# oxylusengine/Oxylus

Measured on NVIDIA H100. Metric: meshlet_instances_culled_per_s, higher is better.
Workload: dtype f32

## Files before the change

### oxylus_b200/csrc/kernels_cull.cuh

```cuda
#pragma once
#include "oxc_filtered.cuh"
#include "oxc_tma.cuh"

namespace oxc {

#ifndef OXC_CULL_MESHES_THREADS
#define OXC_CULL_MESHES_THREADS 64
#endif
constexpr int CULL_MESHES_THREADS = OXC_CULL_MESHES_THREADS;
constexpr int CULL_THREADS = 256;
#ifndef OXC_CULL_ITEMS
#define OXC_CULL_ITEMS 2
#endif
#ifndef OXC_CULL_MIN_BLOCKS
#define OXC_CULL_MIN_BLOCKS 3
#endif
constexpr int CULL_ITEMS = OXC_CULL_ITEMS;
constexpr int CULL_TILE = CULL_THREADS * CULL_ITEMS;

struct MeshesParams {
  const OxcMesh* meshes;
  OxcMeshInstance* mesh_instances;
  const OxcTransformWorld* transforms;
  InstCull* inst;
  InstGeom* geom;
  const float* lod_aabb;
  uint32_t* counts;
  uint32_t* block_sums;
  uint32_t first, count;
  uint32_t flags;
  int select;
  OxcCullCamera cam;
  const OxcCullCamera* cam_dev;
};

__global__ void __launch_bounds__(CULL_MESHES_THREADS) k_cull_meshes(const __grid_constant__ MeshesParams pp) {
  const MeshesParams& p = pp;
  const OxcCullCamera& cam = pp.cam_dev ? *pp.cam_dev : pp.cam;
  const uint32_t local = blockIdx.x * CULL_MESHES_THREADS + threadIdx.x;
  uint32_t meshlet_count = 0;
  if (local < p.count) {
    const uint32_t mi = p.first + local;
    OxcMeshInstance inst = p.mesh_instances[mi];
    const OxcMesh* mesh = &p.meshes[inst.mesh_index];
    const float* world = p.transforms[inst.transform_index].world;
    float w[16];
#pragma unroll
    for (int k = 0; k < 4; k++) {
      const float4 c = __ldg(reinterpret_cast<const float4*>(world) + k);
      w[k * 4 + 0] = c.x; w[k * 4 + 1] = c.y; w[k * 4 + 2] = c.z; w[k * 4 + 3] = c.w;
    }
    float4 rows[4], planes[6];
    mul_mm_rows(cam.projection_view, w, rows);
    frustum_planes(rows, planes);
// ... 68 lines not shown
    if (p.select) {
      InstGeom g;
      g.meshlets = reinterpret_cast<const OxcMeshlet*>(lod->meshlets);
      g.local_triangle_indices = reinterpret_cast<const uint32_t*>(lod->local_triangle_indices);
      g.indirect_vertex_indices = reinterpret_cast<const uint32_t*>(lod->indirect_vertex_indices);
      g.vertex_positions = reinterpret_cast<const uint2*>(mesh->vertex_positions);
      g.vertex_normals = reinterpret_cast<const uint32_t*>(mesh->vertex_normals);
      g.texture_coords = reinterpret_cast<const uint32_t*>(mesh->texture_coords);
      g.transform_index = inst.transform_index;
      g.vertex_count = mesh->vertex_count;
      g.pad[0] = g.pad[1] = 0;
      p.geom[mi] = g;
      p.counts[local] = meshlet_count;
    }
  }
  if (!p.select) return;
  __shared__ uint32_t warp_sums[CULL_MESHES_THREADS / 32];
  uint32_t v = meshlet_count;
#pragma unroll
  for (int o = 16; o > 0; o >>= 1) v += __shfl_xor_sync(0xffffffffu, v, o);
  if ((threadIdx.x & 31) == 0) warp_sums[threadIdx.x >> 5] = v;
  __syncthreads();
  if (threadIdx.x == 0) {
    uint32_t s = 0;
#pragma unroll
    for (int k = 0; k < CULL_MESHES_THREADS / 32; k++) s += warp_sums[k];
    p.block_sums[blockIdx.x] = s;
  }
}

__global__ void __launch_bounds__(CULL_MESHES_THREADS) k_count_prefix_meshlets(const __grid_constant__ MeshesParams p, uint32_t* id_base) {
  const OxcCullCamera& cam = p.cam_dev ? *p.cam_dev : p.cam;
  const uint32_t mi = blockIdx.x * CULL_MESHES_THREADS + threadIdx.x;
  uint32_t meshlet_count = 0;
  if (mi < p.first) {
    const OxcMeshInstance inst = p.mesh_instances[mi];
    const OxcMesh* mesh = &p.meshes[inst.mesh_index];
    const float* world = p.transforms[inst.transform_index].world;
    float w[16];
#pragma unroll
    for (int k = 0; k < 16; k++) w[k] = world[k];
    float4 rows[4], planes[6];
    mul_mm_rows(cam.projection_view, w, rows);
// ... 50 lines not shown
      }
    }
  } else bad = true;
#pragma unroll
  for (int a = 0; a < 3; a++)
#pragma unroll
    for (int o = 16; o > 0; o >>= 1) {
      mn[a] = fminf(mn[a], __shfl_xor_sync(0xffffffffu, mn[a], o));
      mx[a] = fmaxf(mx[a], __shfl_xor_sync(0xffffffffu, mx[a], o));
    }
  bad = __any_sync(0xffffffffu, bad);
  if (lane == 0) {
    float* o = out + (size_t)w * 6;
    if (bad) { o[0] = o[1] = o[2] = 1.0f; o[3] = o[4] = o[5] = -1.0f; }
    else { o[0] = mn[0]; o[1] = mn[1]; o[2] = mn[2]; o[3] = mx[0]; o[4] = mx[1]; o[5] = mx[2]; }
  }
}

__global__ void __launch_bounds__(1024) k_scan_block_sums(uint32_t* block_sums, uint32_t n_blocks,
                                                          OxcMeshletInstanceVisibility* vis,
                                                          OxcDispatchIndirectCommand* cmd, uint32_t capacity, uint32_t* status) {
  __shared__ uint32_t warp_tot[32];
  __shared__ uint32_t carry_s;
  if (threadIdx.x == 0) carry_s = 0;
  __syncthreads();
  for (uint32_t base = 0; base < n_blocks; base += 1024) {
    const uint32_t i = base + threadIdx.x;
    const uint32_t v = i < n_blocks ? block_sums[i] : 0u;
    uint32_t inc = v;
#pragma unroll
    for (int o = 1; o < 32; o <<= 1) {
      const uint32_t t = __shfl_up_sync(0xffffffffu, inc, o);
      if ((threadIdx.x & 31) >= o) inc += t;
    }
    if ((threadIdx.x & 31) == 31) warp_tot[threadIdx.x >> 5] = inc;
    __syncthreads();
    if (threadIdx.x < 32) {
      uint32_t w = warp_tot[threadIdx.x], winc = w;
#pragma unroll
      for (int o = 1; o < 32; o <<= 1) {
        const uint32_t t = __shfl_up_sync(0xffffffffu, winc, o);
        if (threadIdx.x >= o) winc += t;
      }
      warp_tot[threadIdx.x] = winc - w;
    }
    __syncthreads();
    const uint32_t carry = carry_s;
    const uint32_t excl = carry + warp_tot[threadIdx.x >> 5] + inc - v;
    if (i < n_blocks) block_sums[i] = excl;
    __syncthreads();
    if (threadIdx.x == 1023) carry_s = excl + v;
    __syncthreads();
  }
  if (threadIdx.x == 0) {
    uint32_t total = carry_s;
    if (total > capacity) {
      total = capacity;
      atomicOr(status, (uint32_t)OXC_STATUS_MESHLET_OVERFLOW);
    }
    vis->total_visible_meshlet_instances = total;
    vis->early_visible_meshlet_instances = 0;
    vis->late_visible_meshlet_instances = 0;
    cmd->x = (total + 63u) / 64u;
    cmd->y = 1;
    cmd->z = 1;
  }
}

constexpr int EXPAND_SPLIT = 8;
__global__ void __launch_bounds__(CULL_MESHES_THREADS) k_expand_meshlet_instances(const uint32_t* __restrict__ counts,
                                                                                 const uint32_t* __restrict__ block_offsets,
                                                                                 uint32_t first, uint32_t count,
                                                                                 OxcMeshletInstance* out, uint32_t capacity, uint2* slabs) {
  __shared__ uint32_t offs[CULL_MESHES_THREADS];
  __shared__ uint32_t cnts[CULL_MESHES_THREADS];
  __shared__ uint32_t warp_tot[CULL_MESHES_THREADS / 32];
  const uint32_t block = blockIdx.x / EXPAND_SPLIT, part = blockIdx.x % EXPAND_SPLIT;
  const uint32_t local = block * CULL_MESHES_THREADS + threadIdx.x;
  const uint32_t v = local < count ? counts[local] : 0u;
  uint32_t inc = v;
#pragma unroll
  for (int o = 1; o < 32; o <<= 1) {
    const uint32_t t = __shfl_up_sync(0xffffffffu, inc, o);
    if ((threadIdx.x & 31) >= o) inc += t;
  }
  if ((threadIdx.x & 31) == 31) warp_tot[threadIdx.x >> 5] = inc;
  __syncthreads();
  uint32_t wbase = 0;
  for (int k = 0; k < (int)(threadIdx.x >> 5); k++) wbase += warp_tot[k];
  offs[threadIdx.x] = block_offsets[block] + wbase + inc - v;
  cnts[threadIdx.x] = v;
  __syncthreads();
  const uint32_t lane = threadIdx.x & 31, warp = threadIdx.x >> 5;
  uint2* o2 = reinterpret_cast<uint2*>(out);
  constexpr uint32_t PER_PART = CULL_MESHES_THREADS / EXPAND_SPLIT;
  for (uint32_t k = part * PER_PART + warp; k < (part + 1) * PER_PART; k += CULL_MESHES_THREADS / 32) {
    const uint32_t n = cnts[k];
    if (n == 0) continue;
    const uint32_t base = offs[k];
    const uint32_t mi = first + block * CULL_MESHES_THREADS + k;
    for (uint32_t j = lane; j < n && base + j < capacity; j += 32) {
      o2[base + j] = make_uint2(mi, j);
      if (((base + j) & 31u) == 0u) slabs[(base + j) >> 5] = make_uint2(mi, j);
    }
  }
}

constexpr int CULL_WARPS = CULL_THREADS / 32;
constexpr int CULL_Q = 64;
constexpr int CULL_EMIT = 128;
constexpr uint32_t CULL_TILE_BYTES = CULL_TILE * sizeof(OxcMeshletInstance);

template <bool Q0>
struct __align__(16) CullShared {
  uint32_t hiz_off[OXC_HIZ_MAX_LEVELS];
  float s8_lut[256];
  uint4 q0a[CULL_WARPS][Q0 ? CULL_Q : 1];
  uint32_t q0b[CULL_WARPS][Q0 ? CULL_Q : 1];
  uint4 q1a[CULL_WARPS][CULL_Q];
// ... 621 lines not shown
```

### oxylus_b200/csrc/kernels_hiz.cuh

```cuda
#pragma once
#include "oxc_exact.cuh"

namespace oxc {

struct HizBuildParams {
  const float* depth;
  uint32_t elem_stride;
  uint32_t elem_offset;
  uint32_t width, height;
  float* hiz;
  uint32_t hw, hh, levels;
  uint32_t hw_shift, hh_shift;
  uint32_t mode;
  uint32_t level_offset[OXC_HIZ_MAX_LEVELS];
};

OXC_DI float hiz_sample(const HizBuildParams& p, uint32_t x, uint32_t y) {
  uint32_t sx = (uint32_t)(((uint64_t)(x + 1) * p.width) >> p.hw_shift);
  uint32_t sy = (uint32_t)(((uint64_t)(y + 1) * p.height) >> p.hh_shift);
  sx = sx > p.width - 1 ? p.width - 1 : sx;
  sy = sy > p.height - 1 ? p.height - 1 : sy;
  return __ldg(p.depth + ((size_t)sy * p.width + sx) * p.elem_stride + p.elem_offset);
}

__global__ void __launch_bounds__(256) k_hiz_tiles(const __grid_constant__ HizBuildParams p) {
  __shared__ float s2[16][16];
  __shared__ float s3[8][8];
  __shared__ float s4[4][4];
  __shared__ float s5[2][2];
  const uint32_t tx = threadIdx.x & 15, ty = threadIdx.x >> 4;
  const uint32_t x0 = blockIdx.x * 64 + tx * 4, y0 = blockIdx.y * 64 + ty * 4;
  float v[4][4];
#pragma unroll
  for (int j = 0; j < 4; j++)
#pragma unroll
    for (int i = 0; i < 4; i++) v[j][i] = p.mode == 2 ? 0.0f : hiz_sample(p, x0 + i, y0 + j);
  float* m0 = p.hiz + p.level_offset[0];
  if (p.mode == 2) {
#pragma unroll
    for (int j = 0; j < 4; j++) {
      const float4 r = *reinterpret_cast<const float4*>(m0 + (size_t)(y0 + j) * p.hw + x0);
      v[j][0] = r.x; v[j][1] = r.y; v[j][2] = r.z; v[j][3] = r.w;
    }
  } else {
// ... 32 lines not shown
    const float d = omin(omin(s3[2 * y][2 * x], s3[2 * y][2 * x + 1]), omin(s3[2 * y + 1][2 * x], s3[2 * y + 1][2 * x + 1]));
    s4[y][x] = d;
    p.hiz[p.level_offset[4] + (size_t)(blockIdx.y * 4 + y) * (p.hw >> 4) + blockIdx.x * 4 + x] = d;
  }
  __syncthreads();
  if (t < 4) {
    const uint32_t x = t & 1, y = t >> 1;
    const float d = omin(omin(s4[2 * y][2 * x], s4[2 * y][2 * x + 1]), omin(s4[2 * y + 1][2 * x], s4[2 * y + 1][2 * x + 1]));
    s5[y][x] = d;
    p.hiz[p.level_offset[5] + (size_t)(blockIdx.y * 2 + y) * (p.hw >> 5) + blockIdx.x * 2 + x] = d;
  }
  __syncthreads();
  if (t == 0)
    p.hiz[p.level_offset[6] + (size_t)blockIdx.y * (p.hw >> 6) + blockIdx.x] =
        omin(omin(s5[0][0], s5[0][1]), omin(s5[1][0], s5[1][1]));
}

__global__ void __launch_bounds__(1024) k_hiz_tail(const __grid_constant__ HizBuildParams p, uint32_t first_level) {
  for (uint32_t l = first_level; l < p.levels; l++) {
    uint32_t pw = p.hw >> (l - 1), ph = p.hh >> (l - 1), mw = p.hw >> l, mh = p.hh >> l;
    pw = pw < 1 ? 1 : pw; ph = ph < 1 ? 1 : ph; mw = mw < 1 ? 1 : mw; mh = mh < 1 ? 1 : mh;
    const float* src = p.hiz + p.level_offset[l - 1];
    float* dst = p.hiz + p.level_offset[l];
    for (uint32_t i = threadIdx.x; i < mw * mh; i += blockDim.x) {
      const uint32_t x = i % mw, y = i / mw;
      const uint32_t xa = min(2 * x, pw - 1), xb = min(2 * x + 1, pw - 1), ya = min(2 * y, ph - 1), yb = min(2 * y + 1, ph - 1);
      const float a = src[(size_t)ya * pw + xa], b = src[(size_t)ya * pw + xb];
      const float c = src[(size_t)yb * pw + xa], d = src[(size_t)yb * pw + xb];
      dst[i] = omin(omin(a, b), omin(c, d));
    }
    __syncthreads();
  }
}

__global__ void k_hiz_mip0_generic(const __grid_constant__ HizBuildParams p) {
  const uint32_t i = blockIdx.x * blockDim.x + threadIdx.x;
  if (i >= p.hw * p.hh) return;
  p.hiz[p.level_offset[0] + i] = hiz_sample(p, i % p.hw, i / p.hw);
}

__global__ void k_fill_u32(uint32_t* dst, uint32_t value, size_t n) {
  for (size_t i = (size_t)blockIdx.x * blockDim.x + threadIdx.x; i < n; i += (size_t)gridDim.x * blockDim.x) dst[i] = value;
}

}
```

### oxylus_b200/csrc/kernels_tri.cuh

```cuda
#pragma once
#include <climits>

#include "oxc_exact.cuh"
#include "oxc_raster_core.cuh"
#include "oxc_tma.cuh"

namespace oxc {

#ifndef OXC_TRI_THREADS
#define OXC_TRI_THREADS 256
#endif
constexpr int TRI_THREADS = OXC_TRI_THREADS;
constexpr int TRI_WARPS = TRI_THREADS / 32;

struct TriParams {
  const OxcMeshletInstance* meshlet_instances;
  const InstCull* inst;
  const InstGeom* geom;
  const OxcMeshletInstanceVisibility* vis;
  const OxcDispatchIndirectCommand* tri_cmd;
  const uint32_t* visible_indices;
  const uint32_t* id_base;
  uint32_t late;
  uint32_t* reordered_indices;
// ... 520 lines not shown
    const uint32_t g = tile * TRI_WARPS + warp;
    if (g < count) {
      const MeshletWork w = load_meshlet(p, first + g, id_base, clip_s, lane);
      for (uint32_t t = lane; t < w.tri_count; t += 32) {
        float4 c0, c1, c2;
        if (!triangle_passes(w, t, clip_s, c0, c1, c2)) continue;
        if (to_screen(c0, fW, fH).fx != INT_MIN && to_screen(c1, fW, fH).fx != INT_MIN && to_screen(c2, fW, fH).fx != INT_MIN)
          continue;
        clip_and_draw(p, c0, c1, c2, (w.data_id << p.prim_bits) | t, fW, fH);
      }
    }
    __syncwarp();
  }
}

__global__ void k_clear_visbuffer(unsigned long long* vis, size_t n) {
  for (size_t i = (size_t)blockIdx.x * blockDim.x + threadIdx.x; i < n; i += (size_t)gridDim.x * blockDim.x)
    vis[i] = (unsigned long long)OXC_VIS_CLEAR;
}

__global__ void k_clear_visbuffer_depth(unsigned long long* vis, const float* depth, size_t n) {
  for (size_t i = (size_t)blockIdx.x * blockDim.x + threadIdx.x; i < n; i += (size_t)gridDim.x * blockDim.x)
    vis[i] = ((unsigned long long)__float_as_uint(__ldg(&depth[i])) << 32) | OXC_VIS_CLEAR;
}

__global__ void k_merge_depth(unsigned long long* vis, const float* depth, size_t n) {
  for (size_t i = (size_t)blockIdx.x * blockDim.x + threadIdx.x; i < n; i += (size_t)gridDim.x * blockDim.x) {
    const unsigned long long v = ((unsigned long long)__float_as_uint(depth[i]) << 32) | OXC_VIS_CLEAR;
    if (v > vis[i]) vis[i] = v;
  }
}

__global__ void k_resolve_visbuffer(const unsigned long long* vis, uint32_t* vis32, float* depth, size_t n) {
  for (size_t i = (size_t)blockIdx.x * blockDim.x + threadIdx.x; i < n; i += (size_t)gridDim.x * blockDim.x) {
    const unsigned long long v = vis[i];
    if (vis32) vis32[i] = (uint32_t)(v & 0xFFFFFFFFull);
    if (depth) depth[i] = __uint_as_float((uint32_t)(v >> 32));
  }
// ... 4 lines not shown
```

### oxylus_b200/csrc/oxcull.cu

```cuda
#include <cuda_runtime.h>

#include <atomic>
#include <cstdarg>
#include <cstdio>
#include <cstdlib>
#include <cstring>
#include <new>
#include <vector>

#include <dlfcn.h>
#include <nccl.h>

#include "kernels_cull.cuh"
#include "kernels_decode.cuh"
#include "kernels_hiz.cuh"
#include "kernels_mgpu.cuh"
#include "kernels_tri.cuh"
#include "kernels_alpha.cuh"

using namespace oxc;

namespace {

thread_local char g_err[512] = "";
// ... 46 lines not shown
  c->index_count = 0; c->instance_count = 1; c->first_index = 0; c->vertex_offset = 0; c->first_instance = 0;
}
__global__ void k_reset_visibility(OxcMeshletInstanceVisibility* v, OxcDispatchIndirectCommand* c) {
  v->total_visible_meshlet_instances = 0; v->early_visible_meshlet_instances = 0; v->late_visible_meshlet_instances = 0;
  c->x = 0; c->y = 1; c->z = 1;
}

__global__ void k_debug_dequantize(float* canonical, float* hw) {
  const uint32_t h = blockIdx.x * blockDim.x + threadIdx.x;
  if (h < 65536u) { canonical[h] = dequantize_half(h); hw[h] = dequantize_half_hw(h); }
}

uint32_t ilog2(uint32_t v) { uint32_t r = 0; while ((1u << r) < v) r++; return r; }
bool is_pow2(uint32_t v) { return v && !(v & (v - 1)); }

}

struct OxcContext {
  int device = 0;
  int sm_count = 0;
  OxcCreateInfo info{};
  OxcMesh* d_meshes = nullptr;
  OxcMeshInstance* d_mesh_instances = nullptr;
  OxcTransformWorld* d_transforms = nullptr;
  uint8_t* d_blob = nullptr;
  uint32_t mesh_count = 0, mesh_instance_count = 0, transform_count = 0;
  uint32_t mesh_cap = 0, transform_cap = 0;
  uint64_t blob_cap = 0;
  bool scene_set = false;
  InstCull* d_inst = nullptr;
  InstGeom* d_geom = nullptr;
  uint32_t* d_counts = nullptr;
  uint32_t* d_block_sums = nullptr;
  float* d_lod_aabb = nullptr;
  OxcMeshletInstance* d_meshlet_instances = nullptr;
  uint2* d_slabs = nullptr;
  uint32_t* d_visible = nullptr;
  uint32_t* d_mask = nullptr;
  uint32_t mask_words = 0;
  OxcMeshletInstanceVisibility* d_vis = nullptr;
  OxcDispatchIndirectCommand* d_cull_meshlets_cmd = nullptr;
  OxcDispatchIndirectCommand* d_cull_triangles_cmd = nullptr;
  OxcDrawIndexedIndirectCommand* d_draw_cmd = nullptr;
  uint32_t* d_reordered = nullptr;
  unsigned long long* d_tri_counter = nullptr;
  uint32_t* d_raster_work = nullptr;
  uint4* d_big_queue = nullptr;
  uint32_t* d_big_counters = nullptr;
// ... 124 lines not shown
  OxcContext* c = new (std::nothrow) OxcContext();
  if (!c) return fail(OXC_E_INVALID, "out of host memory");
  c->device = device;
  c->info = *info;
  cudaDeviceProp prop;
  CK(cudaGetDeviceProperties(&prop, device));
  c->sm_count = prop.multiProcessorCount;
  const uint32_t I = info->max_mesh_instances ? info->max_mesh_instances : 1;
  const uint32_t N = info->max_meshlet_instances ? info->max_meshlet_instances : 1;
  int rc;
#define TRY(x) if ((rc = (x)) != OXC_OK) { oxc_destroy(c); return rc; }
  TRY(dalloc(&c->d_mesh_instances, (size_t)I));
  TRY(dalloc(&c->d_inst, (size_t)I));
  TRY(dalloc(&c->d_geom, (size_t)I));
  TRY(dalloc(&c->d_counts, (size_t)I));
  TRY(dalloc(&c->d_block_sums, (size_t)(I + CULL_MESHES_THREADS - 1) / CULL_MESHES_THREADS + 1));
  TRY(dalloc(&c->d_meshlet_instances, (size_t)N + CULL_TILE));
  TRY(dalloc(&c->d_slabs, (size_t)N / 32 + 2));
  TRY(dalloc(&c->d_visible, (size_t)N));
  c->mask_words = ((info->max_mask_bits > N ? info->max_mask_bits : N) + 31) / 32;
  TRY(dalloc(&c->d_mask, (size_t)c->mask_words));
  TRY(dalloc(&c->d_vis, 1));
  TRY(dalloc(&c->d_cull_meshlets_cmd, 1));
  TRY(dalloc(&c->d_cull_triangles_cmd, 1));
  TRY(dalloc(&c->d_draw_cmd, 1));
  TRY(dalloc(&c->d_tri_counter, 1));
  TRY(dalloc(&c->d_raster_work, 4));
  c->big_capacity = 1u << 18;
  if (const char* e = getenv("OXC_BIG_CAPACITY")) {
    const long v = atol(e);
    if (v >= 1 && v <= (1l << 24)) c->big_capacity = (uint32_t)v;
// ... 32 lines not shown
        uint32_t mw = info->hiz_width >> l, mh = info->hiz_height >> l;
        off += (mw < 1 ? 1 : mw) * (mh < 1 ? 1 : mh);
      }
    }
    c->hiz.width = info->hiz_width; c->hiz.height = info->hiz_height; c->hiz.levels = levels;
    c->hiz_total = off;
    TRY(dalloc(&c->d_hiz, (size_t)off));
    c->hiz.data = c->d_hiz;
  }
#undef TRY
  CK(cudaMemset(c->d_mask, 0, (size_t)c->mask_words * 4));
  CK(cudaMemset(c->d_hiz, 0, (size_t)c->hiz_total * 4));
  CK(cudaMemset(c->d_vis, 0, sizeof(OxcMeshletInstanceVisibility)));
  CK(cudaMemset(c->d_tri_counter, 0, 8));
  CK(cudaMemset(c->d_status, 0, 4));
  OxcDispatchIndirectCommand one{0, 1, 1};
  CK(cudaMemcpy(c->d_cull_meshlets_cmd, &one, sizeof one, cudaMemcpyHostToDevice));
  CK(cudaMemcpy(c->d_cull_triangles_cmd, &one, sizeof one, cudaMemcpyHostToDevice));
  OxcDrawIndexedIndirectCommand dc{0, 1, 0, 0, 0};
  CK(cudaMemcpy(c->d_draw_cmd, &dc, sizeof dc, cudaMemcpyHostToDevice));
#define OCC(dst, kern, threads) CK(cudaOccupancyMaxActiveBlocksPerMultiprocessor(&(dst), kern, threads, 0))
#define OCCC(dst, H, O, L)                                                                                                        \
  CK(cudaFuncSetAttribute(k_cull_meshlets<H, O, L, false>, cudaFuncAttributeMaxDynamicSharedMemorySize, (int)sizeof(CullShared<O && !L>)));  \
  CK(cudaFuncSetAttribute(k_cull_meshlets<H, O, L, true>, cudaFuncAttributeMaxDynamicSharedMemorySize, (int)sizeof(CullShared<O && !L>)));   \
  CK(cudaOccupancyMaxActiveBlocksPerMultiprocessor(&(dst), (k_cull_meshlets<H, O, L, false>), CULL_THREADS, sizeof(CullShared<O && !L>)))
  OCCC(c->occ_cull[0][0][0], false, false, false);
  OCCC(c->occ_cull[1][0][0], true, false, false);
  OCCC(c->occ_cull[1][0][1], true, false, true);
  OCCC(c->occ_cull[1][1][0], true, true, false);
  OCCC(c->occ_cull[1][1][1], true, true, true);
#undef OCCC
  c->occ_cull[0][0][1] = c->occ_cull[0][1][0] = c->occ_cull[0][1][1] = c->occ_cull[0][0][0];
  OCC(c->occ_tri, k_cull_triangles, TRI_THREADS);
  OCC(c->occ_raster, k_raster_visbuffer<false>, TRI_THREADS);
  OCC(c->occ_mv, k_cull_meshlets_multiview, CULL_THREADS);
#undef OCC
  *out_ctx = c;
  return OXC_OK;
}

void oxc_destroy(OxcContext* c) {
  if (!c) return;
  cudaSetDevice(c->device);
  if (c->mg.active) { cudaDeviceSynchronize(); mgpu_release(c); }
  cudaFree(c->d_meshes); cudaFree(c->d_mesh_instances); cudaFree(c->d_transforms); cudaFree(c->d_blob);
  cudaFree(c->d_lod_aabb); cudaFree(c->d_inst); cudaFree(c->d_geom); cudaFree(c->d_counts); cudaFree(c->d_block_sums);
  cudaFree(c->d_meshlet_instances); cudaFree(c->d_slabs); cudaFree(c->d_visible); cudaFree(c->d_mask); cudaFree(c->d_vis);
  cudaFree(c->d_cull_meshlets_cmd); cudaFree(c->d_cull_triangles_cmd); cudaFree(c->d_draw_cmd);
  cudaFree(c->d_reordered); cudaFree(c->d_tri_counter); cudaFree(c->d_raster_work); cudaFree(c->d_big_queue); cudaFree(c->d_clip_queue); cudaFree(c->d_id_base_auto); cudaFree(c->d_status); cudaFree(c->d_hiz);
  cudaFree(c->d_view_planes); cudaFree(c->d_view_bits); cudaFree(c->d_view_counts); cudaFree(c->d_inst_views);
  cudaFree(c->d_alpha_materials); cudaFree(c->d_alpha_lists); cudaFree(c->d_alpha_cmd);
  delete c;
}

int oxc_set_scene(OxcContext* c, const OxcSceneDesc* sc, void* stream) {
  if (!c || !sc) return fail(OXC_E_INVALID, "null argument");
  cudaStream_t s = static_cast<cudaStream_t>(stream);
  CK(cudaSetDevice(c->device));
  if (sc->mesh_instance_count > c->info.max_mesh_instances)
    return fail(OXC_E_CAPACITY, "mesh_instance_count %u > max_mesh_instances %u", sc->mesh_instance_count, c->info.max_mesh_instances);
  if (sc->mesh_count == 0 || !sc->meshes || !sc->blob || !sc->transforms || (sc->mesh_instance_count && !sc->mesh_instances))
// ... 168 lines not shown
  p.inst = c->d_inst; p.geom = c->d_geom; p.counts = c->d_counts; p.block_sums = c->d_block_sums; p.lod_aabb = c->d_lod_aabb;
  shard_range(c, cam->mesh_instance_count, &p.first, &p.count);
  p.flags = flags; p.select = 1; p.cam = *cam; p.cam_dev = c->cam_dev;
  if (c->id_base_auto) {
    CK(cudaMemsetAsync(c->d_id_base_auto, 0, 4, s));
    if (p.first) {
      k_count_prefix_meshlets<<<(p.first + CULL_MESHES_THREADS - 1) / CULL_MESHES_THREADS, CULL_MESHES_THREADS, 0, s>>>(p, c->d_id_base_auto);
      LAUNCHED();
    }
  }
  const uint32_t n_blocks = (p.count + CULL_MESHES_THREADS - 1) / CULL_MESHES_THREADS;
  if (n_blocks == 0) {
    k_reset_visibility<<<1, 1, 0, s>>>(c->d_vis, c->d_cull_meshlets_cmd);
    LAUNCHED();
  } else {
    k_cull_meshes<<<n_blocks, CULL_MESHES_THREADS, 0, s>>>(p);
    LAUNCHED();
    k_scan_block_sums<<<1, 1024, 0, s>>>(c->d_block_sums, n_blocks, c->d_vis, c->d_cull_meshlets_cmd, c->info.max_meshlet_instances, c->d_status);
    LAUNCHED();
    k_expand_meshlet_instances<<<n_blocks * EXPAND_SPLIT, CULL_MESHES_THREADS, 0, s>>>(c->d_counts, c->d_block_sums, p.first, p.count,
                                                                      c->d_meshlet_instances, c->info.max_meshlet_instances, c->d_slabs);
    LAUNCHED();
  }
  c->cached_cam = *cam;
  c->cache_valid = true;
  return OXC_OK;
}

int oxc_cull_meshlets(OxcContext* c, const OxcCullCamera* cam, uint32_t flags, int use_hiz, void* stream) {
  if (!c || !cam) return fail(OXC_E_INVALID, "null argument");
  if (!c->scene_set) return fail(OXC_E_STATE, "oxc_set_scene first");
  cudaStream_t s = static_cast<cudaStream_t>(stream);
  CK(cudaSetDevice(c->device));
  int rc = refresh_inst_cache(c, cam, s);
  if (rc != OXC_OK) return rc;
  CK(cudaMemsetAsync(&c->d_cull_triangles_cmd->x, 0, 4, s));
// ... 28 lines not shown
#undef GO
  LAUNCHED();
  return OXC_OK;
}

static int build_hiz_impl(OxcContext* c, const float* depth_dev, uint32_t stride, uint32_t offset, uint32_t width,
                          uint32_t height, void* stream, uint32_t mode = 0) {
  if (!c || (!depth_dev && mode != 2) || ((!width || !height) && mode != 2)) return fail(OXC_E_INVALID, "bad argument");
  cudaStream_t s = static_cast<cudaStream_t>(stream);
  CK(cudaSetDevice(c->device));
  HizBuildParams p{};
  p.depth = depth_dev; p.elem_stride = stride; p.elem_offset = offset; p.width = width; p.height = height; p.hiz = c->d_hiz;
  p.hw = c->hiz.width; p.hh = c->hiz.height; p.levels = c->hiz.levels;
  p.hw_shift = ilog2(p.hw); p.hh_shift = ilog2(p.hh);
  p.mode = mode;
  memcpy(p.level_offset, c->hiz.level_offset, sizeof p.level_offset);
  if (p.hw % 64 == 0 && p.hh % 64 == 0) {
    k_hiz_tiles<<<dim3(p.hw / 64, p.hh / 64), 256, 0, s>>>(p);
    LAUNCHED();
    if (p.levels > 7 && mode != 1) { k_hiz_tail<<<1, 1024, 0, s>>>(p, 7); LAUNCHED(); }
  } else {
    const uint32_t n = p.hw * p.hh;
    if (mode != 2) { k_hiz_mip0_generic<<<(n + 255) / 256, 256, 0, s>>>(p); LAUNCHED(); }
    if (p.levels > 1 && mode != 1) { k_hiz_tail<<<1, 1024, 0, s>>>(p, 1); LAUNCHED(); }
  }
  c->hiz_zero = false;
  return OXC_OK;
}

int oxc_build_hiz(OxcContext* c, const float* depth_dev, uint32_t width, uint32_t height, void* stream) {
  return build_hiz_impl(c, depth_dev, 1, 0, width, height, stream);
}

int oxc_build_hiz_packed(OxcContext* c, const uint64_t* vis_dev, uint32_t width, uint32_t height, void* stream) {
  return build_hiz_impl(c, reinterpret_cast<const float*>(vis_dev), 2, 1, width, height, stream);
// ... 42 lines not shown
  LAUNCHED();
  uint32_t tiles = (c->info.max_meshlet_instances + TRI_WARPS - 1) / TRI_WARPS;
  uint32_t grid = (uint32_t)(c->sm_count * (c->occ_tri > 0 ? c->occ_tri : 1));
  if (grid > tiles) grid = tiles;
  if (grid == 0) grid = 1;
  k_cull_triangles<<<grid, TRI_THREADS, 0, s>>>(p);
  LAUNCHED();
  return OXC_OK;
}

int oxc_clear_visbuffer(OxcContext* c, uint64_t* vis, uint32_t w, uint32_t h, void* stream) {
  if (!c || !vis) return fail(OXC_E_INVALID, "null argument");
  cudaStream_t s = static_cast<cudaStream_t>(stream);
  CK(cudaSetDevice(c->device));
  const size_t n = (size_t)w * h;
  k_clear_visbuffer<<<c->sm_count * 8, 256, 0, s>>>(reinterpret_cast<unsigned long long*>(vis), n);
  LAUNCHED();
  CK(cudaMemsetAsync(c->d_tri_counter, 0, 8, s));
  return OXC_OK;
}

int oxc_raster_visbuffer(OxcContext* c, const OxcCullCamera* cam, uint32_t flags, uint32_t w, uint32_t h, uint64_t* vis,
                         int small_primitive_cull, void* stream) {
  if (!c || !cam || !vis) return fail(OXC_E_INVALID, "null argument");
  if (c->scene_id_bound > (1ull << (32u - c->prim_bits)))
    return fail(OXC_E_CAPACITY, "the scene can emit %llu meshlet instances: ids overflow the %u id bits of the vis-buffer word (visbuffer.slang:9-10)%s",
                (unsigned long long)c->scene_id_bound, 32u - c->prim_bits, c->info.wide_ids ? "" : "; create the context with wide_ids = 1 (26 + 6 bit packing)");
  cudaStream_t s = static_cast<cudaStream_t>(stream);
  CK(cudaSetDevice(c->device));
  TriParams p{};
  int rc = tri_common(c, cam, flags, s, &p);
  if (rc != OXC_OK) return rc;
  p.visbuf = reinterpret_cast<unsigned long long*>(vis); p.width = w; p.height = h; p.f_width = (float)w; p.f_height = (float)h;
// ... 168 lines not shown
}

int oxc_resolve_visbuffer(OxcContext* c, const uint64_t* vis, uint32_t w, uint32_t h, uint32_t* vis32, float* depth, void* stream) {
  if (!c || !vis) return fail(OXC_E_INVALID, "null argument");
  cudaStream_t s = static_cast<cudaStream_t>(stream);
  CK(cudaSetDevice(c->device));
  k_resolve_visbuffer<<<c->sm_count * 8, 256, 0, s>>>(reinterpret_cast<const unsigned long long*>(vis), vis32, depth, (size_t)w * h);
  LAUNCHED();
  return OXC_OK;
}

int oxc_clear_visbuffer_with_depth(OxcContext* c, uint64_t* vis, const float* depth_dev, uint32_t w, uint32_t h, void* stream) {
  if (!c || !vis || !depth_dev) return fail(OXC_E_INVALID, "null argument");
  cudaStream_t s = static_cast<cudaStream_t>(stream);
  CK(cudaSetDevice(c->device));
  k_clear_visbuffer_depth<<<c->sm_count * 8, 256, 0, s>>>(reinterpret_cast<unsigned long long*>(vis), depth_dev, (size_t)w * h);
  LAUNCHED();
  CK(cudaMemsetAsync(c->d_tri_counter, 0, 8, s));
  return OXC_OK;
}

int oxc_merge_depth(OxcContext* c, uint64_t* vis, const float* depth_dev, uint32_t w, uint32_t h, void* stream) {
  if (!c || !vis || !depth_dev) return fail(OXC_E_INVALID, "null argument");
  cudaStream_t s = static_cast<cudaStream_t>(stream);
  CK(cudaSetDevice(c->device));
  k_merge_depth<<<c->sm_count * 8, 256, 0, s>>>(reinterpret_cast<unsigned long long*>(vis), depth_dev, (size_t)w * h);
  LAUNCHED();
  return OXC_OK;
}

int oxc_cull_meshlets_multiview(OxcContext* c, const OxcCullCamera* views, uint32_t n_views, int directional, void* stream) {
  if (!c || !views || n_views == 0) return fail(OXC_E_INVALID, "bad argument");
  if (n_views > c->info.max_views || !c->d_view_planes) return fail(OXC_E_CAPACITY, "n_views %u > max_views %u", n_views, c->info.max_views);
// ... 554 lines not shown
```

Before: 1.830 billion.

## Fuse mesh cull, scan and expand into one decoupled-lookback kernel; fold HiZ tail

New measurement: 1.818 billion, median of 6. Within noise of the previous version (-0.7%).

```diff
diff --git a/oxylus_b200/csrc/kernels_cull.cuh b/oxylus_b200/csrc/kernels_cull.cuh
--- a/oxylus_b200/csrc/kernels_cull.cuh
+++ b/oxylus_b200/csrc/kernels_cull.cuh
@@ -28,16 +28,21 @@
   uint32_t* counts;
   uint32_t* block_sums;
   uint32_t first, count;
+  OxcMeshletInstance* meshlet_instances;
+  uint2* slabs;
+  OxcMeshletInstanceVisibility* vis;
+  OxcDispatchIndirectCommand* cmd;
+  uint32_t capacity;
+  uint32_t* status;
+  uint32_t* ctas_done;
   uint32_t flags;
   int select;
   OxcCullCamera cam;
   const OxcCullCamera* cam_dev;
 };
 
-__global__ void __launch_bounds__(CULL_MESHES_THREADS) k_cull_meshes(const __grid_constant__ MeshesParams pp) {
-  const MeshesParams& p = pp;
-  const OxcCullCamera& cam = pp.cam_dev ? *pp.cam_dev : pp.cam;
-  const uint32_t local = blockIdx.x * CULL_MESHES_THREADS + threadIdx.x;
+OXC_DI uint32_t cull_mesh_instance(const MeshesParams& p, uint32_t local) {
+  const OxcCullCamera& cam = p.cam_dev ? *p.cam_dev : p.cam;
   uint32_t meshlet_count = 0;
   if (local < p.count) {
     const uint32_t mi = p.first + local;
@@ -136,19 +141,96 @@
       p.counts[local] = meshlet_count;
     }
   }
-  if (!p.select) return;
-  __shared__ uint32_t warp_sums[CULL_MESHES_THREADS / 32];
-  uint32_t v = meshlet_count;
-#pragma unroll
-  for (int o = 16; o > 0; o >>= 1) v += __shfl_xor_sync(0xffffffffu, v, o);
-  if ((threadIdx.x & 31) == 0) warp_sums[threadIdx.x >> 5] = v;
+  return meshlet_count;
+}
+
+__global__ void __launch_bounds__(CULL_MESHES_THREADS) k_cull_meshes(const __grid_constant__ MeshesParams p) {
+  cull_mesh_instance(p, blockIdx.x * CULL_MESHES_THREADS + threadIdx.x);
+}
+
+constexpr unsigned long long SCAN_AGGREGATE = 1ull << 32, SCAN_PREFIX = 2ull << 32;
+constexpr int EXPAND_THREADS = 8 * CULL_MESHES_THREADS;
+__global__ void __launch_bounds__(EXPAND_THREADS) k_cull_meshes_expand(const __grid_constant__ MeshesParams p) {
+  __shared__ uint32_t offs[CULL_MESHES_THREADS];
+  __shared__ uint32_t cnts[CULL_MESHES_THREADS];
+  __shared__ uint32_t warp_tot[CULL_MESHES_THREADS / 32];
+  __shared__ uint32_t base_s, last_s;
+  const uint32_t lane = threadIdx.x & 31, warp = threadIdx.x >> 5;
+  const uint32_t v = threadIdx.x < (uint32_t)CULL_MESHES_THREADS ? cull_mesh_instance(p, blockIdx.x * CULL_MESHES_THREADS + threadIdx.x) : 0u;
+  uint32_t inc = v;
+#pragma unroll
+  for (int o = 1; o < 32; o <<= 1) {
+    const uint32_t t = __shfl_up_sync(0xffffffffu, inc, o);
+    if (lane >= (uint32_t)o) inc += t;
+  }
+  if (lane == 31 && warp < (uint32_t)CULL_MESHES_THREADS / 32) warp_tot[warp] = inc;
+  __syncthreads();
+  uint32_t wbase = 0, agg = 0;
+#pragma unroll
+  for (int k = 0; k < CULL_MESHES_THREADS / 32; k++) {
+    wbase += (uint32_t)k < warp ? warp_tot[k] : 0u;
+    agg += warp_tot[k];
+  }
+  volatile unsigned long long* look = reinterpret_cast<volatile unsigned long long*>(p.block_sums);
+  if (warp == 0) {
+    if (blockIdx.x > 0 && lane == 0) look[blockIdx.x] = SCAN_AGGREGATE | agg;
+    uint32_t excl = 0;
+    for (int end = (int)blockIdx.x - 1; end >= 0; end -= 32) {
+      const int k = end - (int)lane;
+      unsigned long long s = SCAN_PREFIX;
+      if (k >= 0)
+        while ((s = look[k]) == 0) __nanosleep(20);
+      const uint32_t pre = __ballot_sync(0xffffffffu, (s & SCAN_PREFIX) != 0);
+      const uint32_t stop = pre ? (uint32_t)__ffs(pre) - 1u : 31u;
+      uint32_t add = lane <= stop ? (uint32_t)s : 0u;
+#pragma unroll
+      for (int o = 16; o > 0; o >>= 1) add += __shfl_xor_sync(0xffffffffu, add, o);
+      excl += add;
+      if (pre) break;
+    }
+    if (lane == 0) {
+      look[blockIdx.x] = SCAN_PREFIX | (excl + agg);
+      base_s = excl;
+    }
+  }
+  __syncthreads();
+  if (threadIdx.x < (uint32_t)CULL_MESHES_THREADS) {
+    offs[threadIdx.x] = base_s + wbase + inc - v;
+    cnts[threadIdx.x] = v;
+  }
+  __syncthreads();
+  uint2* o2 = reinterpret_cast<uint2*>(p.meshlet_instances);
+  for (uint32_t k = warp; k < (uint32_t)CULL_MESHES_THREADS; k += EXPAND_THREADS / 32) {
+    const uint32_t n = cnts[k], base = offs[k];
+    const uint32_t mi = p.first + blockIdx.x * CULL_MESHES_THREADS + k;
+    for (uint32_t j = lane; j < n && base + j < p.capacity; j += 32) {
+      o2[base + j] = make_uint2(mi, j);
+      if (((base + j) & 31u) == 0u) p.slabs[(base + j) >> 5] = make_uint2(mi, j);
+    }
+  }
   __syncthreads();
   if (threadIdx.x == 0) {
-    uint32_t s = 0;
-#pragma unroll
-    for (int k = 0; k < CULL_MESHES_THREADS / 32; k++) s += warp_sums[k];
-    p.block_sums[blockIdx.x] = s;
-  }
+    __threadfence();
+    last_s = atomicAdd(p.ctas_done, 1u) == gridDim.x - 1u;
+    if (last_s) {
+      __threadfence();
+      uint32_t total = (uint32_t)look[gridDim.x - 1];
+      if (total > p.capacity) {
+        total = p.capacity;
+        atomicOr(p.status, (uint32_t)OXC_STATUS_MESHLET_OVERFLOW);
+      }
+      p.vis->total_visible_meshlet_instances = total;
+      p.vis->early_visible_meshlet_instances = 0;
+      p.vis->late_visible_meshlet_instances = 0;
+      p.cmd->x = (total + 63u) / 64u;
+      p.cmd->y = 1;
+      p.cmd->z = 1;
+      *p.ctas_done = 0u;
+    }
+  }
+  __syncthreads();
+  if (last_s)
+    for (uint32_t k = threadIdx.x; k < gridDim.x; k += EXPAND_THREADS) look[k] = 0ull;
 }
 
 __global__ void __launch_bounds__(CULL_MESHES_THREADS) k_count_prefix_meshlets(const __grid_constant__ MeshesParams p, uint32_t* id_base) {
@@ -229,95 +311,6 @@
     float* o = out + (size_t)w * 6;
     if (bad) { o[0] = o[1] = o[2] = 1.0f; o[3] = o[4] = o[5] = -1.0f; }
     else { o[0] = mn[0]; o[1] = mn[1]; o[2] = mn[2]; o[3] = mx[0]; o[4] = mx[1]; o[5] = mx[2]; }
-  }
-}
-
-__global__ void __launch_bounds__(1024) k_scan_block_sums(uint32_t* block_sums, uint32_t n_blocks,
-                                                          OxcMeshletInstanceVisibility* vis,
-                                                          OxcDispatchIndirectCommand* cmd, uint32_t capacity, uint32_t* status) {
-  __shared__ uint32_t warp_tot[32];
-  __shared__ uint32_t carry_s;
-  if (threadIdx.x == 0) carry_s = 0;
-  __syncthreads();
-  for (uint32_t base = 0; base < n_blocks; base += 1024) {
-    const uint32_t i = base + threadIdx.x;
-    const uint32_t v = i < n_blocks ? block_sums[i] : 0u;
-    uint32_t inc = v;
-#pragma unroll
-    for (int o = 1; o < 32; o <<= 1) {
-      const uint32_t t = __shfl_up_sync(0xffffffffu, inc, o);
-      if ((threadIdx.x & 31) >= o) inc += t;
-    }
-    if ((threadIdx.x & 31) == 31) warp_tot[threadIdx.x >> 5] = inc;
-    __syncthreads();
-    if (threadIdx.x < 32) {
-      uint32_t w = warp_tot[threadIdx.x], winc = w;
-#pragma unroll
-      for (int o = 1; o < 32; o <<= 1) {
-        const uint32_t t = __shfl_up_sync(0xffffffffu, winc, o);
-        if (threadIdx.x >= o) winc += t;
-      }
-      warp_tot[threadIdx.x] = winc - w;
-    }
-    __syncthreads();
-    const uint32_t carry = carry_s;
-    const uint32_t excl = carry + warp_tot[threadIdx.x >> 5] + inc - v;
-    if (i < n_blocks) block_sums[i] = excl;
-    __syncthreads();
-    if (threadIdx.x == 1023) carry_s = excl + v;
-    __syncthreads();
-  }
-  if (threadIdx.x == 0) {
-    uint32_t total = carry_s;
-    if (total > capacity) {
-      total = capacity;
-      atomicOr(status, (uint32_t)OXC_STATUS_MESHLET_OVERFLOW);
-    }
-    vis->total_visible_meshlet_instances = total;
-    vis->early_visible_meshlet_instances = 0;
-    vis->late_visible_meshlet_instances = 0;
-    cmd->x = (total + 63u) / 64u;
-    cmd->y = 1;
-    cmd->z = 1;
-  }
-}
-
-constexpr int EXPAND_SPLIT = 8;
-__global__ void __launch_bounds__(CULL_MESHES_THREADS) k_expand_meshlet_instances(const uint32_t* __restrict__ counts,
-                                                                                 const uint32_t* __restrict__ block_offsets,
-                                                                                 uint32_t first, uint32_t count,
-                                                                                 OxcMeshletInstance* out, uint32_t capacity, uint2* slabs) {
-  __shared__ uint32_t offs[CULL_MESHES_THREADS];
-  __shared__ uint32_t cnts[CULL_MESHES_THREADS];
-  __shared__ uint32_t warp_tot[CULL_MESHES_THREADS / 32];
-  const uint32_t block = blockIdx.x / EXPAND_SPLIT, part = blockIdx.x % EXPAND_SPLIT;
-  const uint32_t local = block * CULL_MESHES_THREADS + threadIdx.x;
-  const uint32_t v = local < count ? counts[local] : 0u;
-  uint32_t inc = v;
-#pragma unroll
-  for (int o = 1; o < 32; o <<= 1) {
-    const uint32_t t = __shfl_up_sync(0xffffffffu, inc, o);
-    if ((threadIdx.x & 31) >= o) inc += t;
-  }
-  if ((threadIdx.x & 31) == 31) warp_tot[threadIdx.x >> 5] = inc;
-  __syncthreads();
-  uint32_t wbase = 0;
-  for (int k = 0; k < (int)(threadIdx.x >> 5); k++) wbase += warp_tot[k];
-  offs[threadIdx.x] = block_offsets[block] + wbase + inc - v;
-  cnts[threadIdx.x] = v;
-  __syncthreads();
-  const uint32_t lane = threadIdx.x & 31, warp = threadIdx.x >> 5;
-  uint2* o2 = reinterpret_cast<uint2*>(out);
-  constexpr uint32_t PER_PART = CULL_MESHES_THREADS / EXPAND_SPLIT;
-  for (uint32_t k = part * PER_PART + warp; k < (part + 1) * PER_PART; k += CULL_MESHES_THREADS / 32) {
-    const uint32_t n = cnts[k];
-    if (n == 0) continue;
-    const uint32_t base = offs[k];
-    const uint32_t mi = first + block * CULL_MESHES_THREADS + k;
-    for (uint32_t j = lane; j < n && base + j < capacity; j += 32) {
-      o2[base + j] = make_uint2(mi, j);
-      if (((base + j) & 31u) == 0u) slabs[(base + j) >> 5] = make_uint2(mi, j);
-    }
   }
 }
 
diff --git a/oxylus_b200/csrc/kernels_hiz.cuh b/oxylus_b200/csrc/kernels_hiz.cuh
--- a/oxylus_b200/csrc/kernels_hiz.cuh
+++ b/oxylus_b200/csrc/kernels_hiz.cuh
@@ -12,8 +12,26 @@
   uint32_t hw, hh, levels;
   uint32_t hw_shift, hh_shift;
   uint32_t mode;
+  uint32_t* tiles_done;
   uint32_t level_offset[OXC_HIZ_MAX_LEVELS];
 };
+
+OXC_DI void hiz_tail(const HizBuildParams& p, uint32_t first_level) {
+  for (uint32_t l = first_level; l < p.levels; l++) {
+    uint32_t pw = p.hw >> (l - 1), ph = p.hh >> (l - 1), mw = p.hw >> l, mh = p.hh >> l;
+    pw = pw < 1 ? 1 : pw; ph = ph < 1 ? 1 : ph; mw = mw < 1 ? 1 : mw; mh = mh < 1 ? 1 : mh;
+    const float* src = p.hiz + p.level_offset[l - 1];
+    float* dst = p.hiz + p.level_offset[l];
+    for (uint32_t i = threadIdx.x; i < mw * mh; i += blockDim.x) {
+      const uint32_t x = i % mw, y = i / mw;
+      const uint32_t xa = min(2 * x, pw - 1), xb = min(2 * x + 1, pw - 1), ya = min(2 * y, ph - 1), yb = min(2 * y + 1, ph - 1);
+      const float a = src[(size_t)ya * pw + xa], b = src[(size_t)ya * pw + xb];
+      const float c = src[(size_t)yb * pw + xa], d = src[(size_t)yb * pw + xb];
+      dst[i] = omin(omin(a, b), omin(c, d));
+    }
+    __syncthreads();
+  }
+}
 
 OXC_DI float hiz_sample(const HizBuildParams& p, uint32_t x, uint32_t y) {
   uint32_t sx = (uint32_t)(((uint64_t)(x + 1) * p.width) >> p.hw_shift);
@@ -28,6 +46,7 @@
   __shared__ float s3[8][8];
   __shared__ float s4[4][4];
   __shared__ float s5[2][2];
+  __shared__ uint32_t last_s;
   const uint32_t tx = threadIdx.x & 15, ty = threadIdx.x >> 4;
   const uint32_t x0 = blockIdx.x * 64 + tx * 4, y0 = blockIdx.y * 64 + ty * 4;
   float v[4][4];
@@ -90,24 +109,21 @@
   if (t == 0)
     p.hiz[p.level_offset[6] + (size_t)blockIdx.y * (p.hw >> 6) + blockIdx.x] =
         omin(omin(s5[0][0], s5[0][1]), omin(s5[1][0], s5[1][1]));
+  if (p.levels <= 7) return;
+  __threadfence();
+  __syncthreads();
+  if (t == 0) {
+    const uint32_t n = gridDim.x * gridDim.y;
+    last_s = atomicAdd(p.tiles_done, 1u) == n - 1u;
+    if (last_s) *p.tiles_done = 0u;
+  }
+  __syncthreads();
+  if (!last_s) return;
+  __threadfence();
+  hiz_tail(p, 7);
 }
 
-__global__ void __launch_bounds__(1024) k_hiz_tail(const __grid_constant__ HizBuildParams p, uint32_t first_level) {
-  for (uint32_t l = first_level; l < p.levels; l++) {
-    uint32_t pw = p.hw >> (l - 1), ph = p.hh >> (l - 1), mw = p.hw >> l, mh = p.hh >> l;
-    pw = pw < 1 ? 1 : pw; ph = ph < 1 ? 1 : ph; mw = mw < 1 ? 1 : mw; mh = mh < 1 ? 1 : mh;
-    const float* src = p.hiz + p.level_offset[l - 1];
-    float* dst = p.hiz + p.level_offset[l];
-    for (uint32_t i = threadIdx.x; i < mw * mh; i += blockDim.x) {
-      const uint32_t x = i % mw, y = i / mw;
-      const uint32_t xa = min(2 * x, pw - 1), xb = min(2 * x + 1, pw - 1), ya = min(2 * y, ph - 1), yb = min(2 * y + 1, ph - 1);
-      const float a = src[(size_t)ya * pw + xa], b = src[(size_t)ya * pw + xb];
-      const float c = src[(size_t)yb * pw + xa], d = src[(size_t)yb * pw + xb];
-      dst[i] = omin(omin(a, b), omin(c, d));
-    }
-    __syncthreads();
-  }
-}
+__global__ void __launch_bounds__(1024) k_hiz_tail(const __grid_constant__ HizBuildParams p, uint32_t first_level) { hiz_tail(p, first_level); }
 
 __global__ void k_hiz_mip0_generic(const __grid_constant__ HizBuildParams p) {
   const uint32_t i = blockIdx.x * blockDim.x + threadIdx.x;
diff --git a/oxylus_b200/csrc/kernels_tri.cuh b/oxylus_b200/csrc/kernels_tri.cuh
--- a/oxylus_b200/csrc/kernels_tri.cuh
+++ b/oxylus_b200/csrc/kernels_tri.cuh
@@ -558,14 +558,22 @@
   }
 }
 
-__global__ void k_clear_visbuffer(unsigned long long* vis, size_t n) {
-  for (size_t i = (size_t)blockIdx.x * blockDim.x + threadIdx.x; i < n; i += (size_t)gridDim.x * blockDim.x)
-    vis[i] = (unsigned long long)OXC_VIS_CLEAR;
-}
-
-__global__ void k_clear_visbuffer_depth(unsigned long long* vis, const float* depth, size_t n) {
-  for (size_t i = (size_t)blockIdx.x * blockDim.x + threadIdx.x; i < n; i += (size_t)gridDim.x * blockDim.x)
-    vis[i] = ((unsigned long long)__float_as_uint(__ldg(&depth[i])) << 32) | OXC_VIS_CLEAR;
+__global__ void k_clear_visbuffer(unsigned long long* vis, const float* depth, size_t n, unsigned long long* tri_counter) {
+  const size_t tid = (size_t)blockIdx.x * blockDim.x + threadIdx.x, stride = (size_t)gridDim.x * blockDim.x;
+  if (tid == 0) *tri_counter = 0ull;
+  const bool vec = ((reinterpret_cast<size_t>(vis) & 15u) | (reinterpret_cast<size_t>(depth) & 7u)) == 0;
+  const size_t n2 = vec ? n / 2 : 0;
+  for (size_t i = tid; i < n2; i += stride) {
+    uint4 v = make_uint4(OXC_VIS_CLEAR, 0u, OXC_VIS_CLEAR, 0u);
+    if (depth) {
+      const float2 d = __ldg(reinterpret_cast<const float2*>(depth) + i);
+      v.y = __float_as_uint(d.x);
+      v.w = __float_as_uint(d.y);
+    }
+    reinterpret_cast<uint4*>(vis)[i] = v;
+  }
+  for (size_t i = 2 * n2 + tid; i < n; i += stride)
+    vis[i] = ((unsigned long long)(depth ? __float_as_uint(__ldg(&depth[i])) : 0u) << 32) | OXC_VIS_CLEAR;
 }
 
 __global__ void k_merge_depth(unsigned long long* vis, const float* depth, size_t n) {
diff --git a/oxylus_b200/csrc/oxcull.cu b/oxylus_b200/csrc/oxcull.cu
--- a/oxylus_b200/csrc/oxcull.cu
+++ b/oxylus_b200/csrc/oxcull.cu
@@ -84,6 +84,8 @@
 uint32_t ilog2(uint32_t v) { uint32_t r = 0; while ((1u << r) < v) r++; return r; }
 bool is_pow2(uint32_t v) { return v && !(v & (v - 1)); }
 
+enum { TICKET_CULL_MESHES, TICKET_HIZ, TICKET_COUNT };
+
 }
 
 struct OxcContext {
@@ -102,6 +104,7 @@
   InstGeom* d_geom = nullptr;
   uint32_t* d_counts = nullptr;
   uint32_t* d_block_sums = nullptr;
+  uint32_t* d_tickets = nullptr;
   float* d_lod_aabb = nullptr;
   OxcMeshletInstance* d_meshlet_instances = nullptr;
   uint2* d_slabs = nullptr;
@@ -256,7 +259,8 @@
   TRY(dalloc(&c->d_inst, (size_t)I));
   TRY(dalloc(&c->d_geom, (size_t)I));
   TRY(dalloc(&c->d_counts, (size_t)I));
-  TRY(dalloc(&c->d_block_sums, (size_t)(I + CULL_MESHES_THREADS - 1) / CULL_MESHES_THREADS + 1));
+  TRY(dalloc(&c->d_block_sums, 2 * ((size_t)(I + CULL_MESHES_THREADS - 1) / CULL_MESHES_THREADS + 1)));
+  TRY(dalloc(&c->d_tickets, (size_t)TICKET_COUNT));
   TRY(dalloc(&c->d_meshlet_instances, (size_t)N + CULL_TILE));
   TRY(dalloc(&c->d_slabs, (size_t)N / 32 + 2));
   TRY(dalloc(&c->d_visible, (size_t)N));
@@ -319,6 +323,8 @@
   CK(cudaMemset(c->d_vis, 0, sizeof(OxcMeshletInstanceVisibility)));
   CK(cudaMemset(c->d_tri_counter, 0, 8));
   CK(cudaMemset(c->d_status, 0, 4));
+  CK(cudaMemset(c->d_block_sums, 0, 8 * ((size_t)(I + CULL_MESHES_THREADS - 1) / CULL_MESHES_THREADS + 1)));
+  CK(cudaMemset(c->d_tickets, 0, 4 * TICKET_COUNT));
   OxcDispatchIndirectCommand one{0, 1, 1};
   CK(cudaMemcpy(c->d_cull_meshlets_cmd, &one, sizeof one, cudaMemcpyHostToDevice));
   CK(cudaMemcpy(c->d_cull_triangles_cmd, &one, sizeof one, cudaMemcpyHostToDevice));
@@ -349,7 +355,7 @@
   cudaSetDevice(c->device);
   if (c->mg.active) { cudaDeviceSynchronize(); mgpu_release(c); }
   cudaFree(c->d_meshes); cudaFree(c->d_mesh_instances); cudaFree(c->d_transforms); cudaFree(c->d_blob);
-  cudaFree(c->d_lod_aabb); cudaFree(c->d_inst); cudaFree(c->d_geom); cudaFree(c->d_counts); cudaFree(c->d_block_sums);
+  cudaFree(c->d_lod_aabb); cudaFree(c->d_inst); cudaFree(c->d_geom); cudaFree(c->d_counts); cudaFree(c->d_block_sums); cudaFree(c->d_tickets);
   cudaFree(c->d_meshlet_instances); cudaFree(c->d_slabs); cudaFree(c->d_visible); cudaFree(c->d_mask); cudaFree(c->d_vis);
   cudaFree(c->d_cull_meshlets_cmd); cudaFree(c->d_cull_triangles_cmd); cudaFree(c->d_draw_cmd);
   cudaFree(c->d_reordered); cudaFree(c->d_tri_counter); cudaFree(c->d_raster_work); cudaFree(c->d_big_queue); cudaFree(c->d_clip_queue); cudaFree(c->d_id_base_auto); cudaFree(c->d_status); cudaFree(c->d_hiz);
@@ -548,12 +554,9 @@
     k_reset_visibility<<<1, 1, 0, s>>>(c->d_vis, c->d_cull_meshlets_cmd);
     LAUNCHED();
   } else {
-    k_cull_meshes<<<n_blocks, CULL_MESHES_THREADS, 0, s>>>(p);
-    LAUNCHED();
-    k_scan_block_sums<<<1, 1024, 0, s>>>(c->d_block_sums, n_blocks, c->d_vis, c->d_cull_meshlets_cmd, c->info.max_meshlet_instances, c->d_status);
-    LAUNCHED();
-    k_expand_meshlet_instances<<<n_blocks * EXPAND_SPLIT, CULL_MESHES_THREADS, 0, s>>>(c->d_counts, c->d_block_sums, p.first, p.count,
-                                                                      c->d_meshlet_instances, c->info.max_meshlet_instances, c->d_slabs);
+    p.meshlet_instances = c->d_meshlet_instances; p.slabs = c->d_slabs; p.vis = c->d_vis; p.cmd = c->d_cull_meshlets_cmd;
+    p.capacity = c->info.max_meshlet_instances; p.status = c->d_status; p.ctas_done = c->d_tickets + TICKET_CULL_MESHES;
+    k_cull_meshes_expand<<<n_blocks, EXPAND_THREADS, 0, s>>>(p);
     LAUNCHED();
   }
   c->cached_cam = *cam;
@@ -612,11 +615,11 @@
   p.hw = c->hiz.width; p.hh = c->hiz.height; p.levels = c->hiz.levels;
   p.hw_shift = ilog2(p.hw); p.hh_shift = ilog2(p.hh);
   p.mode = mode;
+  p.tiles_done = c->d_tickets + TICKET_HIZ;
   memcpy(p.level_offset, c->hiz.level_offset, sizeof p.level_offset);
   if (p.hw % 64 == 0 && p.hh % 64 == 0) {
     k_hiz_tiles<<<dim3(p.hw / 64, p.hh / 64), 256, 0, s>>>(p);
     LAUNCHED();
-    if (p.levels > 7 && mode != 1) { k_hiz_tail<<<1, 1024, 0, s>>>(p, 7); LAUNCHED(); }
   } else {
     const uint32_t n = p.hw * p.hh;
     if (mode != 2) { k_hiz_mip0_generic<<<(n + 255) / 256, 256, 0, s>>>(p); LAUNCHED(); }
@@ -689,9 +692,8 @@
   cudaStream_t s = static_cast<cudaStream_t>(stream);
   CK(cudaSetDevice(c->device));
   const size_t n = (size_t)w * h;
-  k_clear_visbuffer<<<c->sm_count * 8, 256, 0, s>>>(reinterpret_cast<unsigned long long*>(vis), n);
-  LAUNCHED();
-  CK(cudaMemsetAsync(c->d_tri_counter, 0, 8, s));
+  k_clear_visbuffer<<<c->sm_count * 8, 256, 0, s>>>(reinterpret_cast<unsigned long long*>(vis), nullptr, n, c->d_tri_counter);
+  LAUNCHED();
   return OXC_OK;
 }
 
@@ -890,9 +892,8 @@
   if (!c || !vis || !depth_dev) return fail(OXC_E_INVALID, "null argument");
   cudaStream_t s = static_cast<cudaStream_t>(stream);
   CK(cudaSetDevice(c->device));
-  k_clear_visbuffer_depth<<<c->sm_count * 8, 256, 0, s>>>(reinterpret_cast<unsigned long long*>(vis), depth_dev, (size_t)w * h);
-  LAUNCHED();
-  CK(cudaMemsetAsync(c->d_tri_counter, 0, 8, s));
+  k_clear_visbuffer<<<c->sm_count * 8, 256, 0, s>>>(reinterpret_cast<unsigned long long*>(vis), depth_dev, (size_t)w * h, c->d_tri_counter);
+  LAUNCHED();
   return OXC_OK;
 }
 
```
